# yinyajun/Details-In-Recommendation

Hardware: AMD Instinct MI355X
Metric: CTR samples/sec (embedding gather + FM 2nd-order, 26-field batch 65536) (higher is better)
Workload: dtype f32; 1 GPU; deepfm_gather_fm; batch=65536, fields=26, vocab_per_field=1000000, dim=16, ids=uniform, id_layout=bf, row_policy=auto, parallelism=single GPU, tables resident (1.66 GB)

## Files before the change

### details-in-recommendation_amd/csrc/bag_row.hpp

```cpp
#pragma once
#include "common.hpp"

namespace dir {

template <int VEC> struct VecT;
template <> struct VecT<4> { using T = float4; };
template <> struct VecT<1> { using T = float; };

__device__ __forceinline__ float4 ldv(const float* p, float4*) { return *reinterpret_cast<const float4*>(p); }
__device__ __forceinline__ float ldv(const float* p, float*) { return *p; }
typedef float f32x4_t __attribute__((ext_vector_type(4)));
__device__ __forceinline__ float4 ldv_nt(const float* p, float4*) {
    f32x4_t v = __builtin_nontemporal_load(reinterpret_cast<const f32x4_t*>(p));
    return make_float4(v.x, v.y, v.z, v.w);
}
__device__ __forceinline__ float ldv_nt(const float* p, float*) { return __builtin_nontemporal_load(p); }
__device__ __forceinline__ void stv(float* p, float4 v) { *reinterpret_cast<float4*>(p) = v; }
__device__ __forceinline__ void stv(float* p, float v) { *p = v; }
__device__ __forceinline__ float4 vzero(float4*) { return make_float4(0.f, 0.f, 0.f, 0.f); }
__device__ __forceinline__ float vzero(float*) { return 0.f; }
__device__ __forceinline__ float4 vadd(float4 a, float4 b) { return make_float4(a.x + b.x, a.y + b.y, a.z + b.z, a.w + b.w); }
__device__ __forceinline__ float vadd(float a, float b) { return a + b; }
__device__ __forceinline__ float4 vmul(float4 a, float4 b) { return make_float4(a.x * b.x, a.y * b.y, a.z * b.z, a.w * b.w); }
__device__ __forceinline__ float vmul(float a, float b) { return a * b; }
__device__ __forceinline__ float4 vscale(float4 a, float s) { return make_float4(a.x * s, a.y * s, a.z * s, a.w * s); }
__device__ __forceinline__ float vscale(float a, float s) { return a * s; }
__device__ __forceinline__ float4 vdiv(float4 a, float s) { return make_float4(a.x / s, a.y / s, a.z / s, a.w / s); }
__device__ __forceinline__ float vdiv(float a, float s) { return a / s; }
__device__ __forceinline__ float hadd_into(float acc, float4 v) { return (((acc + v.x) + v.y) + v.z) + v.w; }
__device__ __forceinline__ float hadd_into(float acc, float v) { return acc + v; }

__device__ __forceinline__ uint64_t id_bound(const int64_t* __restrict__ vocab, int f) {
    return vocab ? (uint64_t)vocab[f] : (uint64_t)1 << 63;
}

template <int LPS, typename V>
__device__ __forceinline__ float fm_tail(V sum, V sq, int lane, int c) {
    V sm = vmul(sum, sum);
    V d;
    if constexpr (sizeof(V) == 16) {
        d = make_float4(sm.x - sq.x, sm.y - sq.y, sm.z - sq.z, sm.w - sq.w);
    } else {
        d = sm - sq;
    }
    float acc = 0.f;
    const int gbase = lane & ~(LPS - 1);
#pragma unroll
    for (int cc = 0; cc < LPS; ++cc) {
        float carry = __shfl(acc, gbase + (cc > 0 ? cc - 1 : 0), 64);
        if (c == cc) acc = hadd_into(cc == 0 ? 0.f : carry, d);
    }
    return 0.5f * acc;
}

template <int LPS, typename V>
__device__ __forceinline__ V clip_row(V row, float max_norm, int lane, int c) {
    V sq = vmul(row, row);
    float acc = 0.f;
    const int gbase = lane & ~(LPS - 1);
#pragma unroll
    for (int cc = 0; cc < LPS; ++cc) {
        float carry = __shfl(acc, gbase + (cc > 0 ? cc - 1 : 0), 64);
        if (c == cc) acc = hadd_into(cc == 0 ? 0.f : carry, sq);
    }
    const float l2sum = __shfl(acc, gbase + LPS - 1, 64);
    const float l2norm = l2sum > 0.f ? sqrtf(l2sum) : l2sum;
    return vdiv(vscale(row, max_norm), fmaxf(l2norm, max_norm));
}

}
```

### details-in-recommendation_amd/csrc/embedding_bag.hip

```cpp
#include "common.hpp"
#include "bag_row.hpp"

namespace dir {

template <int LPS, int VEC, int KT, int UF, bool DO_FM, bool DO_OUT, bool NT>
__global__ __launch_bounds__(256) void gather_onehot_k(const float* const* __restrict__ tables,
                                                       const int64_t* __restrict__ vocab,
                                                       const int64_t* __restrict__ ids, int64_t sb,
                                                       int64_t sf, int F, int Krt, int64_t B,
                                                       float* __restrict__ out, int64_t out_ld,
                                                       float* __restrict__ fm) {
    using V = typename VecT<VEC>::T;
    constexpr int SPW = 64 / LPS;
    const int K = KT > 0 ? KT : Krt;
    const int lane = threadIdx.x & 63;
    const int c = lane & (LPS - 1);
    const int s = lane / LPS;
    const int kv = (K + VEC - 1) / VEC;
    const bool cact = c < kv;
    const int64_t nwave = (int64_t)gridDim.x * (blockDim.x >> 6);
    for (int64_t g = (int64_t)blockIdx.x * (blockDim.x >> 6) + (threadIdx.x >> 6); g * SPW < B; g += nwave) {
        const int64_t b = g * SPW + s;
        const bool act = cact && (b < B);
        const int64_t* idp = ids + (act ? b * sb : 0);
        float* op = DO_OUT ? out + (act ? b * out_ld : 0) + c * VEC : nullptr;
        V sum = vzero((V*)nullptr), sq = vzero((V*)nullptr);
        for (int f0 = 0; f0 < F; f0 += UF) {
            int64_t id[UF];
#pragma unroll
            for (int u = 0; u < UF; ++u) {
                const int f = f0 + u;
                id[u] = (act && f < F) ? idp[(int64_t)f * sf] : (int64_t)-1;
            }
            V row[UF];
#pragma unroll
            for (int u = 0; u < UF; ++u) {
                const int f = f0 + u;
                row[u] = vzero((V*)nullptr);
                if (f < F) {
                    const float* t = tables[f];
                    if ((uint64_t)id[u] < id_bound(vocab, f)) row[u] = NT ? ldv_nt(t + id[u] * K + c * VEC, (V*)nullptr) : ldv(t + id[u] * K + c * VEC, (V*)nullptr);
                }
            }
#pragma unroll
            for (int u = 0; u < UF; ++u) {
                const int f = f0 + u;
                if (f < F) {
                    if (DO_OUT && act) stv(op + (int64_t)f * K, row[u]);
                    if (DO_FM) {
                        sum = vadd(sum, row[u]);
                        sq = vadd(sq, vmul(row[u], row[u]));
                    }
                }
            }
        }
        if (DO_FM) {
            float r = fm_tail<LPS>(sum, sq, lane, c);
            if (c == LPS - 1 && b < B) fm[b] = r;
        }
    }
}

template <int LPS, int UF, bool NT>
__global__ __launch_bounds__(256) void gather_packed_rows_k(const float* const* __restrict__ tables,
                                                            const int64_t* __restrict__ vocab,
                                                            const int64_t* __restrict__ ids, int64_t sb, int64_t sf,
                                                            int F, int K, int64_t ld, int lin_col, int64_t B,
                                                            float* __restrict__ out, int64_t out_ld,
                                                            float* __restrict__ fm, const float* __restrict__ bias,
                                                            float* __restrict__ lin_out,
                                                            float* __restrict__ fsum ,
                                                            unsigned int* __restrict__ row_bits = nullptr ,
                                                            unsigned int* __restrict__ all_bits = nullptr ,
                                                            unsigned int* __restrict__ block_bits = nullptr, unsigned int* __restrict__ ticket = nullptr) {
    constexpr int SPW = 64 / LPS;
    const int lane = threadIdx.x & 63;
    const int c = lane & (LPS - 1);
    const int s = lane / LPS;
    const int kv = K >> 2;
    const bool cact = c < kv;
    const bool want_lin = lin_out != nullptr && lin_col >= 0;
    const int cl = want_lin ? (lin_col >> 2) : -1;
    const bool line = cl >= kv && cl < LPS;
    const int lw_lane = line ? cl : 0;
    const bool lact = line ? (c * 4 + 4 <= ld) : cact;
    const int64_t nwave = (int64_t)gridDim.x * (blockDim.x >> 6);
    float wmx = 0.f;
    for (int64_t g = (int64_t)blockIdx.x * (blockDim.x >> 6) + (threadIdx.x >> 6); g * SPW < B; g += nwave) {
        const int64_t b = g * SPW + s;
        const bool act = cact && (b < B);
        const bool ldact = lact && (b < B);
        const int64_t* idp = ids + (ldact ? b * sb : 0);
        float* op = out ? out + (act ? b * out_ld : 0) + c * 4 : nullptr;
        float4 sum = make_float4(0.f, 0.f, 0.f, 0.f), sq = sum;
        float lin = 0.f;
        float4 mx4 = make_float4(0.f, 0.f, 0.f, 0.f);
        for (int f0 = 0; f0 < F; f0 += UF) {
            int64_t id[UF];
#pragma unroll
            for (int u = 0; u < UF; ++u) {
                const int f = f0 + u;
                id[u] = (ldact && f < F) ? idp[(int64_t)f * sf] : (int64_t)-1;
            }
            float4 row[UF];
            float lw[UF];
#pragma unroll
            for (int u = 0; u < UF; ++u) {
                const int f = f0 + u;
                row[u] = make_float4(0.f, 0.f, 0.f, 0.f);
                lw[u] = 0.f;
                if (f < F && (uint64_t)id[u] < id_bound(vocab, f)) {
                    const float* t = tables[f] + id[u] * ld;
                    row[u] = NT ? ldv_nt(t + c * 4, (float4*)nullptr) : ldv(t + c * 4, (float4*)nullptr);
                    if (want_lin && !line && c == 0) lw[u] = NT ? ldv_nt(t + lin_col, (float*)nullptr) : t[lin_col];
                }
            }
            if (line) {
#pragma unroll
                for (int u = 0; u < UF; ++u) {
                    const int e = lin_col & 3;
                    lw[u] = c == cl ? (e == 0 ? row[u].x : e == 1 ? row[u].y : e == 2 ? row[u].z : row[u].w) : 0.f;
                    if (!cact) row[u] = make_float4(0.f, 0.f, 0.f, 0.f);
                }
            }
#pragma unroll
            for (int u = 0; u < UF; ++u) {
                const int f = f0 + u;
                if (f < F) {
                    if (op && act) stv(op + (int64_t)f * K, row[u]);
                    sum = vadd(sum, row[u]);
                    sq = vadd(sq, vmul(row[u], row[u]));
                    lin = lin + lw[u];
                    if (row_bits)
                        mx4 = make_float4(fmaxf(mx4.x, fabsf(row[u].x)), fmaxf(mx4.y, fabsf(row[u].y)), fmaxf(mx4.z, fabsf(row[u].z)),
                                          fmaxf(mx4.w, fabsf(row[u].w)));
                }
            }
        }
        if (row_bits) {
            float mx = fmaxf(fmaxf(mx4.x, mx4.y), fmaxf(mx4.z, mx4.w));
#pragma unroll
            for (int o = LPS >> 1; o > 0; o >>= 1) mx = fmaxf(mx, __shfl_xor(mx, o, 64));
            if (c == 0 && b < B) row_bits[b] = __builtin_bit_cast(unsigned int, mx);
            wmx = fmaxf(wmx, (b < B) ? mx : 0.f);
        }
        if (fsum && act) stv(fsum + b * K + c * 4, sum);
        if (fm) {
            const float r = fm_tail<LPS>(sum, sq, lane, c);
            if (c == LPS - 1 && b < B) fm[b] = r;
        }
        if (want_lin && c == lw_lane && b < B) lin_out[b] = lin + (bias ? bias[0] : 0.f);
    }
    if (all_bits) grid_max_bits(wmx, all_bits, block_bits, ticket);
}

template <int LPS, int VEC, bool CLIP>
__global__ __launch_bounds__(256) void bag_csr_k(const float* const* __restrict__ tables,
                                                 const int64_t* __restrict__ vocab,
                                                 const int64_t* __restrict__ ids,
                                                 const int64_t* __restrict__ offsets ,
                                                 const float* __restrict__ weights, int64_t sb, int64_t sf,
                                                 int F, int K, int64_t B, const int32_t* __restrict__ slot_combiner,
                                                 int combiner, const float* __restrict__ slot_max_norm, float max_norm, int flags,
                                                 float* __restrict__ out, int64_t out_ld) {
    using V = typename VecT<VEC>::T;
    constexpr int SPW = 64 / LPS;
    constexpr int U = 8;
    const int lane = threadIdx.x & 63;
    const int c = lane & (LPS - 1);
    const int s = lane / LPS;
    const int kv = (K + VEC - 1) / VEC;
    const bool cact = c < kv;
    const bool prune_w = (flags & DIR_BAG_PRUNE_NONPOSITIVE_WEIGHTS) != 0;
    const bool nt = (flags & DIR_GATHER_STREAM_ROWS) != 0;
    const int64_t nwave = (int64_t)gridDim.x * (blockDim.x >> 6);
    for (int64_t g = (int64_t)blockIdx.x * (blockDim.x >> 6) + (threadIdx.x >> 6); g * SPW < B; g += nwave) {
        const int64_t b = g * SPW + s;
        const bool sact = b < B;
        const bool act = cact && sact;
        auto load_off = [&](int f, int64_t& beg, int64_t& end) {
            beg = 0;
            end = 0;
            if (sact && f < F) {
                const int64_t bag = b * sb + (int64_t)f * sf;
                if (offsets) {
                    beg = offsets[bag];
                    end = offsets[bag + 1];
                } else {
                    beg = bag;
                    end = bag + 1;
                }
            }
        };
        auto load_ent = [&](int64_t e0, int64_t end, int f, int64_t (&id)[U], float (&w)[U]) {
            const uint64_t bound = f < F ? id_bound(vocab, f) : 0;
#pragma unroll
            for (int u = 0; u < U; ++u) {
                const int64_t e = e0 + u;
                id[u] = e < end ? ids[e] : (int64_t)-1;
                w[u] = (weights && e < end) ? weights[e] : 1.0f;
                if (!((uint64_t)id[u] < bound)) id[u] = -1;
                if (weights && prune_w && !(w[u] > 0.0f)) id[u] = -1;
            }
        };
        int64_t beg0, end0, beg1, end1, beg2, end2;
        int64_t id0[U], id1[U];
        float w0[U], w1[U];
        load_off(0, beg0, end0);
        load_off(1, beg1, end1);
        load_ent(beg0, end0, 0, id0, w0);
        for (int f = 0; f < F; ++f) {
            const float* t = tables[f];
            const int comb = slot_combiner ? slot_combiner[f] : combiner;
            const float mn = slot_max_norm ? slot_max_norm[f] : max_norm;
            load_off(f + 2, beg2, end2);
            load_ent(beg1, end1, f + 1, id1, w1);
            V acc = vzero((V*)nullptr);
            float wsum = 0.f, w2sum = 0.f;
            int cnt = 0;
            for (int64_t e0 = beg0; e0 < end0; e0 += U) {
                if (e0 != beg0) load_ent(e0, end0, f, id0, w0);
                V row[U];
#pragma unroll
                for (int u = 0; u < U; ++u) {
                    row[u] = vzero((V*)nullptr);
                    if (id0[u] >= 0 && cact) row[u] = nt ? ldv_nt(t + id0[u] * K + c * VEC, (V*)nullptr) : ldv(t + id0[u] * K + c * VEC, (V*)nullptr);
                }
                if (CLIP && mn > 0.f) {
#pragma unroll
                    for (int u = 0; u < U; ++u) row[u] = clip_row<LPS>(row[u], mn, lane, c);
                }
#pragma unroll
                for (int u = 0; u < U; ++u) {
                    if (id0[u] >= 0) {
                        acc = weights ? vadd(acc, vscale(row[u], w0[u])) : vadd(acc, row[u]);
                        wsum = wsum + w0[u];
                        w2sum = w2sum + w0[u] * w0[u];
                        ++cnt;
                    }
                }
            }
            if (cnt > 0) {
                if (comb == DIR_COMBINER_MEAN) {
                    acc = vdiv(acc, weights ? wsum : (float)cnt);
                } else if (comb == DIR_COMBINER_SQRTN) {
                    acc = vdiv(acc, weights ? sqrtf(w2sum) : sqrtf((float)cnt));
                }
            }
            if (act) stv(out + b * out_ld + (int64_t)f * K + c * VEC, acc);
            beg0 = beg1; end0 = end1; beg1 = beg2; end1 = end2;
#pragma unroll
            for (int u = 0; u < U; ++u) { id0[u] = id1[u]; w0[u] = w1[u]; }
        }
    }
}

template <int LPS, int VEC>
__global__ __launch_bounds__(256) void fm_k(const float* __restrict__ emb, int64_t ld, int64_t B, int F,
                                            int K, float* __restrict__ out) {
    using V = typename VecT<VEC>::T;
    constexpr int SPW = 64 / LPS;
    const int lane = threadIdx.x & 63;
    const int c = lane & (LPS - 1);
    const int s = lane / LPS;
    const int kv = (K + VEC - 1) / VEC;
    const bool cact = c < kv;
    const int64_t nwave = (int64_t)gridDim.x * (blockDim.x >> 6);
    for (int64_t g = (int64_t)blockIdx.x * (blockDim.x >> 6) + (threadIdx.x >> 6); g * SPW < B; g += nwave) {
        const int64_t b = g * SPW + s;
        const bool act = cact && (b < B);
        const float* ep = emb + (act ? b * ld : 0) + c * VEC;
        V sum = vzero((V*)nullptr), sq = vzero((V*)nullptr);
#pragma unroll 8
        for (int f = 0; f < F; ++f) {
            V r = act ? ldv(ep + (int64_t)f * K, (V*)nullptr) : vzero((V*)nullptr);
            sum = vadd(sum, r);
            sq = vadd(sq, vmul(r, r));
        }
        float r = fm_tail<LPS>(sum, sq, lane, c);
        if (c == LPS - 1 && b < B) out[b] = r;
    }
}

__global__ void check_ids_k(const int64_t* __restrict__ vocab, int F, const int64_t* __restrict__ ids,
                            const int64_t* __restrict__ offsets, int64_t sb, int64_t sf, int64_t B,
                            int32_t* __restrict__ bad) {
    const int64_t n = B * F;
    int local = 0;
    for (int64_t i = (int64_t)blockIdx.x * blockDim.x + threadIdx.x; i < n; i += (int64_t)gridDim.x * blockDim.x) {
        const int64_t b = i / F;
        const int f = (int)(i - b * F);
        const int64_t v = vocab[f];
        if (!offsets) {
            const int64_t id = ids[b * sb + f * sf];
            if (id >= v || id < -1) ++local;
        } else {
            const int64_t bag = b * sb + f * sf;
            for (int64_t e = offsets[bag]; e < offsets[bag + 1]; ++e)
                if (ids[e] >= v || ids[e] < -1) ++local;
        }
    }
    if (local) atomicAdd(bad, local);
}

static int next_pow2(int v) {
    int p = 1;
    while (p < v) p <<= 1;
    return p;
}

static int env_int(const char* name, int dflt) {
    const char* e = getenv(name);
    return e ? atoi(e) : dflt;
}

template <int LPS, int VEC, int KT, bool DO_FM, bool DO_OUT>
static void launch_onehot_uf(int uf, bool stream_rows, int64_t work_blocks, hipStream_t st, const float* const* tables,
                             const int64_t* vocab, const int64_t* ids, int64_t sb, int64_t sf, int F, int K, int64_t B, float* out,
                             int64_t out_ld, float* fm) {
    static const int nt_force = env_int("DIR_GATHER_NT", -1);
    const bool nt_env = nt_force >= 0 ? nt_force != 0 : stream_rows;
#define DIR_GO(UF)                                                                                                  \
    do {                                                                                                            \
        if (nt_env) {                                                                                               \
            dim3 grid(grid_resident(work_blocks, resident_blocks(gather_onehot_k<LPS, VEC, KT, UF, DO_FM, DO_OUT, true>))); \
            hipLaunchKernelGGL((gather_onehot_k<LPS, VEC, KT, UF, DO_FM, DO_OUT, true>), grid, dim3(256), 0, st, tables, vocab, ids, sb, sf, F, K, B, out, out_ld, fm); \
        } else {                                                                                                    \
            dim3 grid(grid_resident(work_blocks, resident_blocks(gather_onehot_k<LPS, VEC, KT, UF, DO_FM, DO_OUT, false>))); \
            hipLaunchKernelGGL((gather_onehot_k<LPS, VEC, KT, UF, DO_FM, DO_OUT, false>), grid, dim3(256), 0, st, tables, vocab, ids, sb, sf, F, K, B, out, out_ld, fm); \
        }                                                                                                           \
    } while (0)
    switch (uf) {
        case 4: DIR_GO(4); break;
        case 13: DIR_GO(13); break;
        case 26: DIR_GO(26); break;
        default: DIR_GO(8); break;
    }
#undef DIR_GO
}

template <bool DO_FM, bool DO_OUT>
static int launch_onehot(const float* const* tables, const int64_t* vocab, int F, int K, const int64_t* ids, int64_t sb, int64_t sf,
                         int flags, int64_t B, float* out, int64_t out_ld, float* fm, hipStream_t st) {
    const bool vec = (K % 4 == 0) && (!DO_OUT || (out_ld % 4 == 0 && aligned16(out)));
    static const int uf_env = env_int("DIR_GATHER_UF", 0);
    int uf = uf_env > 0 ? uf_env : (F == 26 ? 26 : (F % 13 == 0 ? 13 : (F > 48 ? 26 : 8)));
    const bool stream_rows = (flags & DIR_GATHER_STREAM_ROWS) != 0;
    const int lps = next_pow2(vec ? K / 4 : K);
    if (lps > 64) return fail(DIR_E_UNSUPPORTED, "embedding row of K=%d floats is wider than one wave covers (max %d)", K, vec ? 256 : 64);
    const int spw = 64 / lps;
    const int64_t waves = (B + spw - 1) / spw;
    const int64_t grid = (waves + 3) / 4;
#define DIR_CASE(L, V, KT) launch_onehot_uf<L, V, KT, DO_FM, DO_OUT>(uf, stream_rows, grid, st, tables, vocab, ids, sb, sf, F, K, B, out, out_ld, fm)
    if (vec) {
        switch (lps) {
            case 1: DIR_CASE(1, 4, 4); break;
            case 2: if (K == 8) DIR_CASE(2, 4, 8); else DIR_CASE(2, 4, 0); break;
            case 4: if (K == 16) DIR_CASE(4, 4, 16); else DIR_CASE(4, 4, 0); break;
            case 8: if (K == 32) DIR_CASE(8, 4, 32); else DIR_CASE(8, 4, 0); break;
            case 16: if (K == 64) DIR_CASE(16, 4, 64); else DIR_CASE(16, 4, 0); break;
            case 32: DIR_CASE(32, 4, 0); break;
            default: DIR_CASE(64, 4, 0); break;
        }
    } else {
        switch (lps) {
            case 1: DIR_CASE(1, 1, 1); break;
            case 2: DIR_CASE(2, 1, 0); break;
            case 4: DIR_CASE(4, 1, 0); break;
            case 8: DIR_CASE(8, 1, 0); break;
            case 16: DIR_CASE(16, 1, 0); break;
            case 32: DIR_CASE(32, 1, 0); break;
            default: DIR_CASE(64, 1, 0); break;
        }
    }
#undef DIR_CASE
    DIR_CHECK_LAUNCH("gather_onehot");
    return DIR_OK;
}

static int launch_csr(const float* const* tables, const int64_t* vocab, int F, int K, const int64_t* ids, const int64_t* offsets,
                      const float* weights, int64_t sb, int64_t sf, const int32_t* slot_combiner, int combiner, const float* slot_max_norm,
                      float max_norm, int flags, int64_t B, float* out, int64_t out_ld, hipStream_t st) {
    const bool vec = (K % 4 == 0) && (out_ld % 4 == 0) && aligned16(out);
    const int lps = next_pow2(vec ? K / 4 : K);
    if (lps > 64) return fail(DIR_E_UNSUPPORTED, "embedding row of K=%d floats is wider than one wave covers", K);
    const int spw = 64 / lps;
    const int64_t waves = (B + spw - 1) / spw;
    dim3 grid(grid_for((waves + 3) / 4));
#define DIR_CASE(L, V)                                                                                                              \
    do {                                                                                                                            \
        if (max_norm > 0.f || slot_max_norm)                                                                                        \
            hipLaunchKernelGGL((bag_csr_k<L, V, true>), grid, dim3(256), 0, st, tables, vocab, ids, offsets, weights, sb, sf, F, K, B, \
                               slot_combiner, combiner, slot_max_norm, max_norm, flags, out, out_ld);                               \
        else                                                                                                                        \
            hipLaunchKernelGGL((bag_csr_k<L, V, false>), grid, dim3(256), 0, st, tables, vocab, ids, offsets, weights, sb, sf, F, K, B, \
                               slot_combiner, combiner, slot_max_norm, max_norm, flags, out, out_ld);                               \
    } while (0)
    if (vec) {
        switch (lps) {
            case 1: DIR_CASE(1, 4); break;
            case 2: DIR_CASE(2, 4); break;
            case 4: DIR_CASE(4, 4); break;
            case 8: DIR_CASE(8, 4); break;
            case 16: DIR_CASE(16, 4); break;
            case 32: DIR_CASE(32, 4); break;
            default: DIR_CASE(64, 4); break;
        }
    } else {
        switch (lps) {
            case 1: DIR_CASE(1, 1); break;
            case 2: DIR_CASE(2, 1); break;
            case 4: DIR_CASE(4, 1); break;
            case 8: DIR_CASE(8, 1); break;
            case 16: DIR_CASE(16, 1); break;
            case 32: DIR_CASE(32, 1); break;
            default: DIR_CASE(64, 1); break;
        }
    }
#undef DIR_CASE
    DIR_CHECK_LAUNCH("bag_csr");
    return DIR_OK;
}

}

using namespace dir;

extern "C" int dir_embedding_bag_ex2_f32(const float* const* tables, const int64_t* vocab, int F, int K, const int64_t* ids,
                                         const int64_t* offsets, const float* weights, int64_t stride_b, int64_t stride_f,
                                         const int32_t* slot_combiner, int combiner, const float* slot_max_norm, float max_norm, int flags,
                                         int64_t B, float* out, int64_t out_ld, dir_stream_t stream) {
    DIR_CHECK_ARG(F > 0 && K > 0 && B >= 0, "dir_embedding_bag_f32: F=%d K=%d B=%lld", F, K, (long long)B);
    if (B == 0) return DIR_OK;
    DIR_CHECK_ARG(tables && ids && out, "dir_embedding_bag_f32: null pointer");
    DIR_CHECK_ARG(out_ld >= (int64_t)F * K, "dir_embedding_bag_f32: out_ld=%lld < F*K=%lld", (long long)out_ld, (long long)F * K);
    DIR_CHECK_ARG(combiner >= DIR_COMBINER_SUM && combiner <= DIR_COMBINER_SQRTN, "dir_embedding_bag_f32: combiner=%d", combiner);
    DIR_CHECK_ARG(offsets || !weights, "dir_embedding_bag_f32: weights need offsets (multi-hot)");
    DIR_CHECK_ARG(!(max_norm < 0.f), "dir_embedding_bag_f32: max_norm=%g", max_norm);
    if (!offsets && !(max_norm > 0.f) && !slot_max_norm)
        return launch_onehot<false, true>(tables, vocab, F, K, ids, stride_b, stride_f, flags, B, out, out_ld, nullptr, as_stream(stream));
    return launch_csr(tables, vocab, F, K, ids, offsets, weights, stride_b, stride_f, slot_combiner, combiner, slot_max_norm, max_norm, flags, B,
                      out, out_ld, as_stream(stream));
}

extern "C" int dir_embedding_bag_ex_f32(const float* const* tables, const int64_t* vocab, int F, int K, const int64_t* ids,
                                        const int64_t* offsets, const float* weights, int64_t stride_b, int64_t stride_f,
                                        const int32_t* slot_combiner, int combiner, float max_norm, int flags, int64_t B,
                                        float* out, int64_t out_ld, dir_stream_t stream) {
    return dir_embedding_bag_ex2_f32(tables, vocab, F, K, ids, offsets, weights, stride_b, stride_f, slot_combiner, combiner, nullptr, max_norm,
                                     flags, B, out, out_ld, stream);
}

extern "C" int dir_embedding_bag_f32(const float* const* tables, int F, int K, const int64_t* ids,
                                     const int64_t* offsets, const float* weights, int64_t stride_b,
                                     int64_t stride_f, int combiner, int flags, int64_t B, float* out,
                                     int64_t out_ld, dir_stream_t stream) {
    return dir_embedding_bag_ex_f32(tables, nullptr, F, K, ids, offsets, weights, stride_b, stride_f, nullptr, combiner, 0.f, flags, B,
                                    out, out_ld, stream);
}

extern "C" int dir_gather_fm_fused_f32(const float* const* tables, const int64_t* vocab, int F, int K, const int64_t* ids,
                                       int64_t stride_b, int64_t stride_f, int flags, int64_t B, float* out,
                                       int64_t out_ld, float* fm, dir_stream_t stream) {
    DIR_CHECK_ARG(F > 0 && K > 0 && B >= 0, "dir_gather_fm_fused_f32: F=%d K=%d B=%lld", F, K, (long long)B);
    if (B == 0) return DIR_OK;
    DIR_CHECK_ARG(tables && ids && (out || fm), "dir_gather_fm_fused_f32: null pointer");
    DIR_CHECK_ARG(!out || out_ld >= (int64_t)F * K, "dir_gather_fm_fused_f32: out_ld=%lld < F*K", (long long)out_ld);
    hipStream_t st = as_stream(stream);
    if (out && fm) return launch_onehot<true, true>(tables, vocab, F, K, ids, stride_b, stride_f, flags, B, out, out_ld, fm, st);
    if (fm) return launch_onehot<true, false>(tables, vocab, F, K, ids, stride_b, stride_f, flags, B, nullptr, 0, fm, st);
    return launch_onehot<false, true>(tables, vocab, F, K, ids, stride_b, stride_f, flags, B, out, out_ld, nullptr, st);
}

extern "C" int dir_fm_second_order_f32(const float* emb, int64_t emb_ld, int64_t B, int F, int K, float* out,
                                       dir_stream_t stream) {
    DIR_CHECK_ARG(emb && out, "dir_fm_second_order_f32: null pointer");
    DIR_CHECK_ARG(F > 0 && K > 0 && B >= 0 && emb_ld >= (int64_t)F * K, "dir_fm_second_order_f32: F=%d K=%d B=%lld ld=%lld", F, K, (long long)B, (long long)emb_ld);
    if (B == 0) return DIR_OK;
    const bool vec = (K % 4 == 0) && (emb_ld % 4 == 0) && aligned16(emb);
    const int lps = next_pow2(vec ? K / 4 : K);
    if (lps > 64) return fail(DIR_E_UNSUPPORTED, "dir_fm_second_order_f32: K=%d too wide", K);
    const int spw = 64 / lps;
    const int64_t waves = (B + spw - 1) / spw;
    dim3 grid(grid_for((waves + 3) / 4));
    hipStream_t st = as_stream(stream);
#define DIR_CASE(L, V) hipLaunchKernelGGL((fm_k<L, V>), grid, dim3(256), 0, st, emb, emb_ld, B, F, K, out)
    if (vec) {
        switch (lps) {
            case 1: DIR_CASE(1, 4); break;
            case 2: DIR_CASE(2, 4); break;
            case 4: DIR_CASE(4, 4); break;
            case 8: DIR_CASE(8, 4); break;
            case 16: DIR_CASE(16, 4); break;
            case 32: DIR_CASE(32, 4); break;
            default: DIR_CASE(64, 4); break;
        }
    } else {
        switch (lps) {
            case 1: DIR_CASE(1, 1); break;
            case 2: DIR_CASE(2, 1); break;
            case 4: DIR_CASE(4, 1); break;
            case 8: DIR_CASE(8, 1); break;
            case 16: DIR_CASE(16, 1); break;
            case 32: DIR_CASE(32, 1); break;
            default: DIR_CASE(64, 1); break;
        }
    }
#undef DIR_CASE
    DIR_CHECK_LAUNCH("fm_second_order");
    return DIR_OK;
}

extern "C" int dir_check_ids(const int64_t* vocab, int F, const int64_t* ids, const int64_t* offsets,
                             int64_t stride_b, int64_t stride_f, int64_t B, int32_t* bad_count,
                             dir_stream_t stream) {
    DIR_CHECK_ARG(vocab && ids && bad_count && F > 0 && B >= 0, "dir_check_ids: bad argument");
    hipStream_t st = as_stream(stream);
    if (zero_async(bad_count, sizeof(int32_t), st) != hipSuccess) return fail(DIR_E_HIP, "dir_check_ids: memset failed");
    if (B == 0) return DIR_OK;
    dim3 grid(grid_for((B * F + 255) / 256));
    hipLaunchKernelGGL(check_ids_k, grid, dim3(256), 0, st, vocab, F, ids, offsets, stride_b, stride_f, B, bad_count);
    DIR_CHECK_LAUNCH("check_ids");
    return DIR_OK;
}

static int gather_packed_launch(const float* const* tables, const int64_t* vocab, int F, int K, int64_t ld, int lin_col,
                                const int64_t* ids, int64_t stride_b, int64_t stride_f, int flags,
                                int64_t B, float* out, int64_t out_ld, float* fm, const float* bias,
                                float* lin_out, float* fsum, dir_stream_t stream, unsigned int* row_bits = nullptr,
                                unsigned int* all_bits = nullptr, unsigned int* bits_ws = nullptr) {
    DIR_CHECK_ARG(F > 0 && K > 0 && B >= 0 && ld >= K && lin_col < ld, "dir_gather_fm_linear_packed_f32: F=%d K=%d ld=%lld lin_col=%d", F, K, (long long)ld, lin_col);
    if (B == 0) return DIR_OK;
    DIR_CHECK_ARG(tables && ids && (out || fm || lin_out || fsum), "dir_gather_fm_linear_packed_f32: null pointer");
    DIR_CHECK_ARG(!out || out_ld >= (int64_t)F * K, "dir_gather_fm_linear_packed_f32: out_ld");
    if ((K & 3) || (ld & 3) || (out && ((out_ld & 3) || !aligned16(out))))
        return fail(DIR_E_UNSUPPORTED, "dir_gather_fm_linear_packed_f32: K, ld, out_ld must be multiples of 4 and out 16-byte aligned");
    int lps = next_pow2(K / 4);
    if (lps > 16) return fail(DIR_E_UNSUPPORTED, "dir_gather_fm_linear_packed_f32: K=%d (supported: up to 64)", K);
    if (lin_out && lin_col >= K && next_pow2(lin_col / 4 + 1) == 2 * lps && 2 * lps <= 16) lps *= 2;
    const int spw = 64 / lps;
    const int64_t waves = (B + spw - 1) / spw;
    const int64_t work = (waves + 3) / 4;
    const bool nt = (flags & DIR_GATHER_STREAM_ROWS) != 0;
    hipStream_t st = as_stream(stream);
#define DIR_GO(L, NTV)                                                                                          \
    do {                                                                                                        \
        dim3 grid(grid_resident(work, resident_blocks(gather_packed_rows_k<L, 13, NTV>)));                     \
        hipLaunchKernelGGL((gather_packed_rows_k<L, 13, NTV>), grid, dim3(256), 0, st, tables, vocab, ids, stride_b, stride_f, F, K, ld, \
                           lin_col, B, out, out_ld, fm, bias, lin_out, fsum, row_bits, all_bits, bits_ws ? bits_ws + 1 : nullptr, bits_ws); \
    } while (0)
#define DIR_L(L) do { if (nt) DIR_GO(L, true); else DIR_GO(L, false); } while (0)
    switch (lps) {
        case 1: DIR_L(1); break;
        case 2: DIR_L(2); break;
        case 4: DIR_L(4); break;
        case 8: DIR_L(8); break;
        default: DIR_L(16); break;
    }
#undef DIR_L
#undef DIR_GO
    DIR_CHECK_LAUNCH("gather_fm_linear_packed");
    return DIR_OK;
}

extern "C" int dir_gather_fm_linear_packed_f32(const float* const* tables, const int64_t* vocab, int F, int K, int64_t ld, int lin_col,
                                               const int64_t* ids, int64_t stride_b, int64_t stride_f, int flags,
                                               int64_t B, float* out, int64_t out_ld, float* fm, const float* bias,
                                               float* lin_out, dir_stream_t stream) {
    return gather_packed_launch(tables, vocab, F, K, ld, lin_col, ids, stride_b, stride_f, flags, B, out, out_ld, fm, bias, lin_out, nullptr, stream);
}

extern "C" int dir_gather_fm_rows_bits_f32(const float* const* tables, const int64_t* vocab, int F, int K, int64_t ld, const int64_t* ids,
                                           int64_t stride_b, int64_t stride_f, int flags, int64_t B, float* out, int64_t out_ld,
                                           float* fm, float* fsum, unsigned int* row_bits, unsigned int* all_bits, unsigned int* workspace,
                                           dir_stream_t stream) {
    DIR_CHECK_ARG(row_bits && all_bits && workspace, "dir_gather_fm_rows_bits_f32: null pointer");
    if (B == 0) {
        if (zero_async(all_bits, sizeof(unsigned int), as_stream(stream)) != hipSuccess) return fail(DIR_E_HIP, "dir_gather_fm_rows_bits_f32: zeroing failed");
        return DIR_OK;
    }
    return gather_packed_launch(tables, vocab, F, K, ld, -1, ids, stride_b, stride_f, flags, B, out, out_ld, fm, nullptr, nullptr, fsum, stream,
                                row_bits, all_bits, workspace);
}

extern "C" int dir_gather_fm_rows_f32(const float* const* tables, const int64_t* vocab, int F, int K, int64_t ld, const int64_t* ids,
                                      int64_t stride_b, int64_t stride_f, int flags, int64_t B, float* out, int64_t out_ld,
                                      float* fm, float* fsum, dir_stream_t stream) {
    return gather_packed_launch(tables, vocab, F, K, ld, -1, ids, stride_b, stride_f, flags, B, out, out_ld, fm, nullptr, nullptr, fsum, stream);
}
```

Before: 1.057 billion samples/s.

## Software-pipeline embedding row gathers with staged table metadata in LDS

Replaces the batched per-field unrolled gather with a rolling software pipeline that prefetches ids one window ahead and row loads one window ahead, with sched barriers and register pinning. Table pointers and vocab bounds are staged once per block in shared memory, and out-of-range ids are redirected to a zero row instead of branching. The default unroll width drops from 26/13 to 8. This aims to keep more independent memory loads in flight and remove per-field scalar pointer loads, at the cost of extra registers and added control complexity.

After: 910.1 million samples/s. 13.9% lower.

```diff
diff --git a/details-in-recommendation_amd/csrc/bag_row.hpp b/details-in-recommendation_amd/csrc/bag_row.hpp
--- a/details-in-recommendation_amd/csrc/bag_row.hpp
+++ b/details-in-recommendation_amd/csrc/bag_row.hpp
@@ -32,6 +32,84 @@
 
 __device__ __forceinline__ uint64_t id_bound(const int64_t* __restrict__ vocab, int f) {
     return vocab ? (uint64_t)vocab[f] : (uint64_t)1 << 63;
+}
+
+#define DIR_AS1 __attribute__((address_space(1)))
+typedef const float DIR_AS1* grow_t;
+constexpr int kStageSlots = 64;
+static __device__ __attribute__((aligned(128))) float dir_zero_row[32] = {0.f};
+
+__device__ __forceinline__ float4 ldg(grow_t p, float4*, bool nt) {
+    const f32x4_t v = nt ? __builtin_nontemporal_load(reinterpret_cast<const f32x4_t DIR_AS1*>(p)) : *reinterpret_cast<const f32x4_t DIR_AS1*>(p);
+    return make_float4(v.x, v.y, v.z, v.w);
+}
+__device__ __forceinline__ float ldg(grow_t p, float*, bool nt) { return nt ? __builtin_nontemporal_load(p) : *p; }
+__device__ __forceinline__ void pin(float4& v) { asm volatile("" : "+v"(v.x), "+v"(v.y), "+v"(v.z), "+v"(v.w)); }
+__device__ __forceinline__ void pin(float& v) { asm volatile("" : "+v"(v)); }
+
+__device__ __forceinline__ void stage_slots(ulonglong2* meta, const float* const* __restrict__ tables, const int64_t* __restrict__ vocab, int f0, int n) {
+    for (int i = threadIdx.x; i < n; i += blockDim.x) meta[i] = make_ulonglong2((unsigned long long)tables[f0 + i], id_bound(vocab, f0 + i));
+}
+
+template <int W, typename V, bool NT, bool LW, typename Use>
+__device__ __forceinline__ void gather_window(const ulonglong2* meta, int fs, int fe, const int64_t* __restrict__ idp, int64_t sf, bool idact,
+                                              int64_t rs, int coff, bool lwact, int lw_col, Use&& use) {
+    unsigned long long zaddr = (unsigned long long)(grow_t)dir_zero_row;
+    asm volatile("" : "+v"(zaddr));
+    const grow_t zero = (grow_t)zaddr;
+    int64_t id[W];
+    V row[W];
+    float lw[W];
+    int f_id = fs, f_row = fs;
+    const int64_t* ip = idp + (int64_t)fs * sf;
+    auto load_id = [&](int u) {
+        id[u] = *ip;
+        ++f_id;
+        if (f_id < fe) ip += sf;
+    };
+    ulonglong2 m = meta[0];
+    auto load_row = [&](int u) {
+        const unsigned long long bound = (idact && f_row < fe) ? m.y : 0ull;
+        const bool ok = (unsigned long long)id[u] < bound;
+        const unsigned long long r = m.x + (unsigned long long)id[u] * (unsigned long long)(rs * 4);
+        row[u] = ldg(ok ? (grow_t)(r + 4ull * coff) : zero, (V*)nullptr, NT);
+        if (LW) lw[u] = ldg((ok && lwact) ? (grow_t)(r + 4ull * lw_col) : zero, (float*)nullptr, NT);
+        ++f_row;
+        m = meta[(f_row < fe ? f_row : fe - 1) - fs];
+    };
+#pragma unroll
+    for (int u = 0; u < W; ++u) load_id(u);
+    const bool second = fs + W < fe;
+#pragma unroll
+    for (int u = 0; u < W; ++u) {
+        load_row(u);
+        if (second) load_id(u);
+        __builtin_amdgcn_sched_barrier(0);
+    }
+    int f0 = fs;
+    for (; f0 + 2 * W < fe; f0 += W) {
+#pragma unroll
+        for (int u = 0; u < W; ++u) {
+            use(f0 + u, row[u], LW ? lw[u] : 0.f, true);
+            load_row(u);
+            load_id(u);
+            __builtin_amdgcn_sched_barrier(0);
+        }
+    }
+    if (f0 + W < fe) {
+#pragma unroll
+        for (int u = 0; u < W; ++u) {
+            use(f0 + u, row[u], LW ? lw[u] : 0.f, true);
+            load_row(u);
+            __builtin_amdgcn_sched_barrier(0);
+        }
+        f0 += W;
+    }
+#pragma unroll
+    for (int u = 0; u < W; ++u) {
+        use(f0 + u, row[u], LW ? lw[u] : 0.f, f0 + u < fe);
+        __builtin_amdgcn_sched_barrier(0);
+    }
 }
 
 template <int LPS, typename V>
diff --git a/details-in-recommendation_amd/csrc/embedding_bag.hip b/details-in-recommendation_amd/csrc/embedding_bag.hip
--- a/details-in-recommendation_amd/csrc/embedding_bag.hip
+++ b/details-in-recommendation_amd/csrc/embedding_bag.hip
@@ -3,7 +3,7 @@
 
 namespace dir {
 
-template <int LPS, int VEC, int KT, int UF, bool DO_FM, bool DO_OUT, bool NT>
+template <int LPS, int VEC, int KT, int W, bool DO_FM, bool DO_OUT, bool NT>
 __global__ __launch_bounds__(256) void gather_onehot_k(const float* const* __restrict__ tables,
                                                        const int64_t* __restrict__ vocab,
                                                        const int64_t* __restrict__ ids, int64_t sb,
@@ -12,47 +12,41 @@
                                                        float* __restrict__ fm) {
     using V = typename VecT<VEC>::T;
     constexpr int SPW = 64 / LPS;
+    __shared__ ulonglong2 meta[kStageSlots];
     const int K = KT > 0 ? KT : Krt;
     const int lane = threadIdx.x & 63;
     const int c = lane & (LPS - 1);
     const int s = lane / LPS;
     const int kv = (K + VEC - 1) / VEC;
     const bool cact = c < kv;
-    const int64_t nwave = (int64_t)gridDim.x * (blockDim.x >> 6);
-    for (int64_t g = (int64_t)blockIdx.x * (blockDim.x >> 6) + (threadIdx.x >> 6); g * SPW < B; g += nwave) {
-        const int64_t b = g * SPW + s;
+    const bool staged_once = F <= kStageSlots;
+    if (staged_once) {
+        stage_slots(meta, tables, vocab, 0, F);
+        __syncthreads();
+    }
+    const int64_t nwork = (B + 4 * SPW - 1) / (4 * SPW);
+    for (int64_t wb = blockIdx.x; wb < nwork; wb += gridDim.x) {
+        const int64_t b = (wb * 4 + (threadIdx.x >> 6)) * SPW + s;
         const bool act = cact && (b < B);
         const int64_t* idp = ids + (act ? b * sb : 0);
         float* op = DO_OUT ? out + (act ? b * out_ld : 0) + c * VEC : nullptr;
         V sum = vzero((V*)nullptr), sq = vzero((V*)nullptr);
-        for (int f0 = 0; f0 < F; f0 += UF) {
-            int64_t id[UF];
-#pragma unroll
-            for (int u = 0; u < UF; ++u) {
-                const int f = f0 + u;
-                id[u] = (act && f < F) ? idp[(int64_t)f * sf] : (int64_t)-1;
+        for (int fs = 0; fs < F; fs += kStageSlots) {
+            const int fe = F - fs < kStageSlots ? F : fs + kStageSlots;
+            if (!staged_once) {
+                __syncthreads();
+                stage_slots(meta, tables, vocab, fs, fe - fs);
+                __syncthreads();
             }
-            V row[UF];
-#pragma unroll
-            for (int u = 0; u < UF; ++u) {
-                const int f = f0 + u;
-                row[u] = vzero((V*)nullptr);
-                if (f < F) {
-                    const float* t = tables[f];
-                    if ((uint64_t)id[u] < id_bound(vocab, f)) row[u] = NT ? ldv_nt(t + id[u] * K + c * VEC, (V*)nullptr) : ldv(t + id[u] * K + c * VEC, (V*)nullptr);
-                }
-            }
-#pragma unroll
-            for (int u = 0; u < UF; ++u) {
-                const int f = f0 + u;
-                if (f < F) {
-                    if (DO_OUT && act) stv(op + (int64_t)f * K, row[u]);
-                    if (DO_FM) {
-                        sum = vadd(sum, row[u]);
-                        sq = vadd(sq, vmul(row[u], row[u]));
-                    }
-                }
-            }
+            gather_window<W, V, NT, false>(meta, fs, fe, idp, sf, act, K, c * VEC, false, 0, [&](int f, V r, float, bool real) {
+                if (DO_OUT && act && real) stv(op + (int64_t)f * K, r);
+                if (DO_FM) {
+                    sum = vadd(sum, r);
+                    sq = vadd(sq, vmul(r, r));
+                    pin(sum);
+                    pin(sq);
+                }
+            });
         }
         if (DO_FM) {
             float r = fm_tail<LPS>(sum, sq, lane, c);
@@ -61,7 +55,7 @@
     }
 }
 
-template <int LPS, int UF, bool NT>
+template <int LPS, int W, bool NT, bool LW>
 __global__ __launch_bounds__(256) void gather_packed_rows_k(const float* const* __restrict__ tables,
                                                             const int64_t* __restrict__ vocab,
                                                             const int64_t* __restrict__ ids, int64_t sb, int64_t sf,
@@ -74,6 +68,7 @@
                                                             unsigned int* __restrict__ all_bits = nullptr ,
                                                             unsigned int* __restrict__ block_bits = nullptr, unsigned int* __restrict__ ticket = nullptr) {
     constexpr int SPW = 64 / LPS;
+    __shared__ ulonglong2 meta[kStageSlots];
     const int lane = threadIdx.x & 63;
     const int c = lane & (LPS - 1);
     const int s = lane / LPS;
@@ -84,10 +79,15 @@
     const bool line = cl >= kv && cl < LPS;
     const int lw_lane = line ? cl : 0;
     const bool lact = line ? (c * 4 + 4 <= ld) : cact;
-    const int64_t nwave = (int64_t)gridDim.x * (blockDim.x >> 6);
+    const bool staged_once = F <= kStageSlots;
+    if (staged_once) {
+        stage_slots(meta, tables, vocab, 0, F);
+        __syncthreads();
+    }
     float wmx = 0.f;
-    for (int64_t g = (int64_t)blockIdx.x * (blockDim.x >> 6) + (threadIdx.x >> 6); g * SPW < B; g += nwave) {
-        const int64_t b = g * SPW + s;
+    const int64_t nwork = (B + 4 * SPW - 1) / (4 * SPW);
+    for (int64_t wb = blockIdx.x; wb < nwork; wb += gridDim.x) {
+        const int64_t b = (wb * 4 + (threadIdx.x >> 6)) * SPW + s;
         const bool act = cact && (b < B);
         const bool ldact = lact && (b < B);
         const int64_t* idp = ids + (ldact ? b * sb : 0);
@@ -95,47 +95,29 @@
         float4 sum = make_float4(0.f, 0.f, 0.f, 0.f), sq = sum;
         float lin = 0.f;
         float4 mx4 = make_float4(0.f, 0.f, 0.f, 0.f);
-        for (int f0 = 0; f0 < F; f0 += UF) {
-            int64_t id[UF];
-#pragma unroll
-            for (int u = 0; u < UF; ++u) {
-                const int f = f0 + u;
-                id[u] = (ldact && f < F) ? idp[(int64_t)f * sf] : (int64_t)-1;
+        for (int fs = 0; fs < F; fs += kStageSlots) {
+            const int fe = F - fs < kStageSlots ? F : fs + kStageSlots;
+            if (!staged_once) {
+                __syncthreads();
+                stage_slots(meta, tables, vocab, fs, fe - fs);
+                __syncthreads();
             }
-            float4 row[UF];
-            float lw[UF];
-#pragma unroll
-            for (int u = 0; u < UF; ++u) {
-                const int f = f0 + u;
-                row[u] = make_float4(0.f, 0.f, 0.f, 0.f);
-                lw[u] = 0.f;
-                if (f < F && (uint64_t)id[u] < id_bound(vocab, f)) {
-                    const float* t = tables[f] + id[u] * ld;
-                    row[u] = NT ? ldv_nt(t + c * 4, (float4*)nullptr) : ldv(t + c * 4, (float4*)nullptr);
-                    if (want_lin && !line && c == 0) lw[u] = NT ? ldv_nt(t + lin_col, (float*)nullptr) : t[lin_col];
-                }
-            }
-            if (line) {
-#pragma unroll
-                for (int u = 0; u < UF; ++u) {
+            gather_window<W, float4, NT, LW>(meta, fs, fe, idp, sf, ldact, ld, c * 4, c == 0, lin_col, [&](int f, float4 r, float w, bool real) {
+                if (line) {
                     const int e = lin_col & 3;
-                    lw[u] = c == cl ? (e == 0 ? row[u].x : e == 1 ? row[u].y : e == 2 ? row[u].z : row[u].w) : 0.f;
-                    if (!cact) row[u] = make_float4(0.f, 0.f, 0.f, 0.f);
-                }
-            }
-#pragma unroll
-            for (int u = 0; u < UF; ++u) {
-                const int f = f0 + u;
-                if (f < F) {
-                    if (op && act) stv(op + (int64_t)f * K, row[u]);
-                    sum = vadd(sum, row[u]);
-                    sq = vadd(sq, vmul(row[u], row[u]));
-                    lin = lin + lw[u];
-                    if (row_bits)
-                        mx4 = make_float4(fmaxf(mx4.x, fabsf(row[u].x)), fmaxf(mx4.y, fabsf(row[u].y)), fmaxf(mx4.z, fabsf(row[u].z)),
-                                          fmaxf(mx4.w, fabsf(row[u].w)));
-                }
-            }
+                    w = c == cl ? (e == 0 ? r.x : e == 1 ? r.y : e == 2 ? r.z : r.w) : 0.f;
+                    if (!cact) r = make_float4(0.f, 0.f, 0.f, 0.f);
+                }
+                if (op && act && real) stv(op + (int64_t)f * K, r);
+                sum = vadd(sum, r);
+                sq = vadd(sq, vmul(r, r));
+                lin = lin + w;
+                pin(sum);
+                pin(sq);
+                pin(lin);
+                if (row_bits)
+                    mx4 = make_float4(fmaxf(mx4.x, fabsf(r.x)), fmaxf(mx4.y, fabsf(r.y)), fmaxf(mx4.z, fabsf(r.z)), fmaxf(mx4.w, fabsf(r.w)));
+            });
         }
         if (row_bits) {
             float mx = fmaxf(fmaxf(mx4.x, mx4.y), fmaxf(mx4.z, mx4.w));
@@ -320,20 +302,19 @@
                              int64_t out_ld, float* fm) {
     static const int nt_force = env_int("DIR_GATHER_NT", -1);
     const bool nt_env = nt_force >= 0 ? nt_force != 0 : stream_rows;
-#define DIR_GO(UF)                                                                                                  \
+#define DIR_GO(W)                                                                                                   \
     do {                                                                                                            \
         if (nt_env) {                                                                                               \
-            dim3 grid(grid_resident(work_blocks, resident_blocks(gather_onehot_k<LPS, VEC, KT, UF, DO_FM, DO_OUT, true>))); \
-            hipLaunchKernelGGL((gather_onehot_k<LPS, VEC, KT, UF, DO_FM, DO_OUT, true>), grid, dim3(256), 0, st, tables, vocab, ids, sb, sf, F, K, B, out, out_ld, fm); \
+            dim3 grid(grid_resident(work_blocks, resident_blocks(gather_onehot_k<LPS, VEC, KT, W, DO_FM, DO_OUT, true>))); \
+            hipLaunchKernelGGL((gather_onehot_k<LPS, VEC, KT, W, DO_FM, DO_OUT, true>), grid, dim3(256), 0, st, tables, vocab, ids, sb, sf, F, K, B, out, out_ld, fm); \
         } else {                                                                                                    \
-            dim3 grid(grid_resident(work_blocks, resident_blocks(gather_onehot_k<LPS, VEC, KT, UF, DO_FM, DO_OUT, false>))); \
-            hipLaunchKernelGGL((gather_onehot_k<LPS, VEC, KT, UF, DO_FM, DO_OUT, false>), grid, dim3(256), 0, st, tables, vocab, ids, sb, sf, F, K, B, out, out_ld, fm); \
+            dim3 grid(grid_resident(work_blocks, resident_blocks(gather_onehot_k<LPS, VEC, KT, W, DO_FM, DO_OUT, false>))); \
+            hipLaunchKernelGGL((gather_onehot_k<LPS, VEC, KT, W, DO_FM, DO_OUT, false>), grid, dim3(256), 0, st, tables, vocab, ids, sb, sf, F, K, B, out, out_ld, fm); \
         }                                                                                                           \
     } while (0)
     switch (uf) {
         case 4: DIR_GO(4); break;
-        case 13: DIR_GO(13); break;
-        case 26: DIR_GO(26); break;
+        case 13: case 26: DIR_GO(13); break;
         default: DIR_GO(8); break;
     }
 #undef DIR_GO
@@ -344,7 +325,7 @@
                          int flags, int64_t B, float* out, int64_t out_ld, float* fm, hipStream_t st) {
     const bool vec = (K % 4 == 0) && (!DO_OUT || (out_ld % 4 == 0 && aligned16(out)));
     static const int uf_env = env_int("DIR_GATHER_UF", 0);
-    int uf = uf_env > 0 ? uf_env : (F == 26 ? 26 : (F % 13 == 0 ? 13 : (F > 48 ? 26 : 8)));
+    const int uf = uf_env > 0 ? uf_env : 8;
     const bool stream_rows = (flags & DIR_GATHER_STREAM_ROWS) != 0;
     const int lps = next_pow2(vec ? K / 4 : K);
     if (lps > 64) return fail(DIR_E_UNSUPPORTED, "embedding row of K=%d floats is wider than one wave covers (max %d)", K, vec ? 256 : 64);
@@ -542,14 +523,20 @@
     const int64_t waves = (B + spw - 1) / spw;
     const int64_t work = (waves + 3) / 4;
     const bool nt = (flags & DIR_GATHER_STREAM_ROWS) != 0;
+    const int cl = lin_col >> 2;
+    const bool lw_sep = lin_out && lin_col >= 0 && !(cl >= (K >> 2) && cl < lps);
     hipStream_t st = as_stream(stream);
-#define DIR_GO(L, NTV)                                                                                          \
+#define DIR_GO(L, NTV, LWV)                                                                                     \
     do {                                                                                                        \
-        dim3 grid(grid_resident(work, resident_blocks(gather_packed_rows_k<L, 13, NTV>)));                     \
-        hipLaunchKernelGGL((gather_packed_rows_k<L, 13, NTV>), grid, dim3(256), 0, st, tables, vocab, ids, stride_b, stride_f, F, K, ld, \
+        dim3 grid(grid_resident(work, resident_blocks(gather_packed_rows_k<L, 8, NTV, LWV>)));                 \
+        hipLaunchKernelGGL((gather_packed_rows_k<L, 8, NTV, LWV>), grid, dim3(256), 0, st, tables, vocab, ids, stride_b, stride_f, F, K, ld, \
                            lin_col, B, out, out_ld, fm, bias, lin_out, fsum, row_bits, all_bits, bits_ws ? bits_ws + 1 : nullptr, bits_ws); \
     } while (0)
-#define DIR_L(L) do { if (nt) DIR_GO(L, true); else DIR_GO(L, false); } while (0)
+#define DIR_L(L)                                                                                                \
+    do {                                                                                                        \
+        if (lw_sep) { if (nt) DIR_GO(L, true, true); else DIR_GO(L, false, true); }                             \
+        else { if (nt) DIR_GO(L, true, false); else DIR_GO(L, false, false); }                                  \
+    } while (0)
     switch (lps) {
         case 1: DIR_L(1); break;
         case 2: DIR_L(2); break;
```
